# TheAustinator/keypoint-consensus-motion-correction

Hardware: AMD Instinct MI355X
Metric: aligned frames/sec (whole node) at 1080p; RANSAC hypotheses scored/sec/GPU (higher is better)
Workload: dtype u16 frames; u8 descriptors: i8 MFMA exact integer distances, f64 RANSAC, f32 warp weights

## Files before the change

keypoint-consensus-motion-correction_amd/csrc/ransac.hip:

```cpp
#include <cfloat>
#include <cmath>

#include "kcmc_internal.h"
#include "ransac_common.h"

namespace kcmc {
namespace {

using namespace ransac_common;

struct Model {
  double c, s, tx, ty;
  bool ok;
};

template <bool SCALE>
__device__ __forceinline__ Model fit2(double sx0, double sy0, double sx1, double sy1, double dx0, double dy0,
                                      double dx1, double dy1) {
  Model m;
  const double ms0 = (sx0 + sx1) / 2.0, ms1 = (sy0 + sy1) / 2.0;
  const double md0 = (dx0 + dx1) / 2.0, md1 = (dy0 + dy1) / 2.0;
  const double a0 = sx0 - ms0, a1 = sy0 - ms1, b0 = sx1 - ms0, b1 = sy1 - ms1;
  const double p0 = dx0 - md0, p1 = dy0 - md1, q0 = dx1 - md0, q1 = dy1 - md1;
  const double a00 = p0 * a0 + q0 * b0;
  const double a01 = p0 * a1 + q0 * b1;
  const double a10 = p1 * a0 + q1 * b0;
  const double a11 = p1 * a1 + q1 * b1;
  const double a = a00 + a11, b = a10 - a01;
  m.ok = !(a == 0.0 && b == 0.0);
  if (SCALE) {
    const double v = (a0 * a0 + b0 * b0) + (a1 * a1 + b1 * b1);
    m.c = a / v;
    m.s = b / v;
  } else {
    const double hn = sqrt(a * a + b * b);
    m.c = a / hn;
    m.s = b / hn;
  }
  m.tx = md0 - (m.c * ms0 - m.s * ms1);
  m.ty = md1 - (m.s * ms0 + m.c * ms1);
  return m;
}

struct Pts {
  const double* sx;
  const double* sy;
  const double* dx;
  const double* dy;
};

__device__ __forceinline__ double resid2(const Model& m, const Pts& P, int k, double thresh, int& cnt) {
  const double x = P.sx[k], y = P.sy[k];
  const double xp = fma(y, -m.s, x * m.c) + m.tx;
  const double yp = fma(y, m.c, x * m.s) + m.ty;
  const double ex = xp - P.dx[k], ey = yp - P.dy[k];
  const double r = sqrt_resid(ex * ex + ey * ey);
  cnt += (r < thresh) ? 1 : 0;
  return r * r;
}

__device__ __forceinline__ float score_fast(const Model& m, const Pts& P, int N, double tq, int& cnt) {
  float S = 0.f;
  for (int k = 0; k < N; ++k) {
    const double x = P.sx[k], y = P.sy[k];
    const double xp = fma(y, -m.s, x * m.c) + m.tx;
    const double yp = fma(y, m.c, x * m.s) + m.ty;
    const double ex = xp - P.dx[k], ey = yp - P.dy[k];
    const double q = ex * ex + ey * ey;
    cnt += (q < tq) ? 1 : 0;
    S += (float)q;
  }
  return S;
}

template <bool LARGE, bool SCALE>
__device__ __forceinline__ void ransac_rigid_frame(
    int f, const double* __restrict__ src, const double* __restrict__ dst, const int32_t* __restrict__ pt_idx,
    const int32_t* __restrict__ pt_off, int src_stride, const uint32_t* __restrict__ hyp,
    const int32_t* __restrict__ hyp_off, int hyp_off_len,
    int T, double thresh, double tq, double rate, int n_skip, double* __restrict__ out_params,
    uint8_t* __restrict__ out_inl, int32_t* __restrict__ out_nin, int32_t* __restrict__ out_best) {
  extern __shared__ __attribute__((aligned(16))) double smem[];
  __shared__ double red[kThreads / 64 * 8];
  __shared__ Scratch sc;
  __shared__ int s_any_zero;
  __shared__ Plan s_plan;

  const int tid = threadIdx.x;
  const int lane = tid & 63, wave = tid >> 6;
  int p0, N, hoff;
  if (!frame_begin<LARGE, 6>(f, pt_off, n_skip, 3, hyp_off, hyp_off_len, out_params, out_inl, out_nin, out_best, p0, N,
                             hoff))
    return;
  const uint32_t* H = hyp + hoff;

  double* sx = smem;
  double* sy = sx + N;
  double* dxs = sy + N;
  double* dys = dxs + N;
  float4* pk32 = reinterpret_cast<float4*>(dys + N);
  double* tS = reinterpret_cast<double*>(pk32 + N);
  double* tSh = tS + T;
  double* stk = tSh + T;
  double* wvals = stk + (LARGE ? kMaxStack * kThreads : 0);
  int* tC = reinterpret_cast<int*>(wvals + kThreads / 64 * 128);
  uint8_t* inl = reinterpret_cast<uint8_t*>(tC + T);
  if (LARGE && tid == 0) {
    s_plan.n = 0;
    plan_gen<kPwDepth>(s_plan, 0, N);
  }

  auto gather = [&](int k, double (&c)[4]) {
    gather_point(src, dst, pt_idx, src_stride, f, p0 + k, c[0], c[1], c[2], c[3]);
  };
  if (tid == 0) s_any_zero = 0;
  __shared__ Mag mg;
  if (!LARGE) {
    if (wave == 0) {
      double c[2][4], lo[4] = {INFINITY, INFINITY, INFINITY, INFINITY}, hi[4] = {-INFINITY, -INFINITY, -INFINITY, -INFINITY};
      bool bad = false;
#pragma unroll
      for (int h = 0; h < 2; ++h) {
        const int k = lane + 64 * h;
        if (k < N) {
          gather(k, c[h]);
          mag_add(c[h], lo, hi, bad);
        }
      }
      wave_bounds(lo, hi, bad);
      const Mag m = mag_of(lo, hi);
      if (lane == 0) mg = m;
#pragma unroll
      for (int h = 0; h < 2; ++h) {
        const int k = lane + 64 * h;
        if (k < N) {
          sx[k] = c[h][0];
          sy[k] = c[h][1];
          dxs[k] = c[h][2];
          dys[k] = c[h][3];
          pk32[k] = centred32(c[h][0], c[h][1], c[h][2], c[h][3], m);
        }
      }
    }
    __syncthreads();
  } else {
    for (int k = tid; k < N; k += kThreads) {
      double c[4];
      gather(k, c);
      sx[k] = c[0];
      sy[k] = c[1];
      dxs[k] = c[2];
      dys[k] = c[3];
    }
    __syncthreads();
    frame_mag(sx, sy, dxs, dys, N, red, mg);
    for (int k = tid; k < N; k += kThreads) pk32[k] = centred32(sx[k], sy[k], dxs[k], dys[k], mg);
    __syncthreads();
  }

  const Pts P{sx, sy, dxs, dys};
  auto fit_of = [&](int t) {
    const uint32_t pr = H[t];
    const int i = (int)(pr & 0xffffu), j = (int)(pr >> 16);
    return fit2<SCALE>(sx[i], sy[i], sx[j], sy[j], dxs[i], dys[i], dxs[j], dys[j]);
  };

  const bool fast = tq == tq;
  int mcount = -1, flag = fast ? 0 : 1;
  if (fast) {
    int mlo = -1;
    bool deferred = false;
    for (int t = tid; t < T; t += kThreads) {
      const Model m = fit_of(t);
      int v = -1;
      double slo = NAN, shi = NAN;
      Lin32 L;
      if (m.ok && lin32_make(m.c, -m.s, m.tx, m.s, m.c, m.ty, mg, tq, L)) {
        int clo = 0, chi = 0;
        const float S32 = score32(pk32, N, L, clo, chi);
        s32_bracket(S32, N, L.be, slo, shi);
        v = pack_cnt(clo, chi - clo);
        if (!(slo >= 1e-30 && shi <= 1e30)) flag = 1;
      } else if (m.ok) {
        v = INT_MIN;
        deferred = true;
      }
      tC[t] = v;
      tS[t] = slo;
      tSh[t] = shi;
      mlo = max(mlo, cnt_of(v));
    }
    if (deferred) {
      for (int t = tid; t < T; t += kThreads) {
        if (tC[t] != INT_MIN) continue;
        const Model m = fit_of(t);
        int cnt = 0;
        const float S32 = score_fast(m, P, N, tq, cnt);
        double slo, shi;
        s64_bracket(S32, N, slo, shi);
        if (!(slo >= 1e-30 && shi <= 1e30)) flag = 1;
        tC[t] = cnt;
        tS[t] = slo;
        tSh[t] = shi;
        mlo = max(mlo, cnt);
      }
    }
    block_max_flag(mlo, flag, sc.cnt);
    __syncthreads();
    for_each_wave_trial(
        T, [&](int t) { return !flag && und_of(tC[t]) > 0 && cnt_of(tC[t]) + und_of(tC[t]) >= mlo; },
        [&](int tc) {
          const Model m = fit_of(tc);
          int c = 0;
          double sq = 0.0;
          for (int k = lane; k < N; k += 64) {
            const double x = sx[k], y = sy[k];
            const double xp = fma(y, -m.s, x * m.c) + m.tx;
            const double yp = fma(y, m.c, x * m.s) + m.ty;
            const double ex = xp - dxs[k], ey = yp - dys[k];
            const double q = ex * ex + ey * ey;
            c += (q < tq) ? 1 : 0;
            sq += q;
          }
          c = wave_sum_i(c);
          double slo, shi;
          sd_bracket(wave_sum(sq), N, slo, shi);
          if (!(slo >= 1e-30 && shi <= 1e30)) flag = 1;
          if (lane == 0) {
            tC[tc] = c;
            tS[tc] = slo;
            tSh[tc] = shi;
          }
        });
    __syncthreads();
    for (int t = tid; t < T; t += kThreads) mcount = max(mcount, cnt_of(tC[t]));
  }
  block_max_flag(mcount, flag, sc.cnt);
  const bool exact = flag != 0 || mcount <= 0;

  Best best;
  bool any_zero = false;
  if (exact) {
    exact_trials(
        T,
        [&](int t, int& cnt) {
          const Model m = fit_of(t);
          if (!m.ok) return (double)NAN;
          return thread_pairwise<LARGE>([&](int k) { return resid2(m, P, k, thresh, cnt); }, N, s_plan, stk, tid);
        },
        tS, tC, best, any_zero);
  } else {
    double lm = INFINITY;
    for (int t = tid; t < T; t += kThreads)
      if (cnt_of(tC[t]) == mcount) lm = fmin(lm, tSh[t]);
    const double minhi = block_min(lm, sc.min);
    double* vals = wvals + wave * 128;
    double* wstk = stk + wave * kMaxStack;
    for_each_wave_trial(
        T, [&](int t) { return cnt_of(tC[t]) == mcount && tS[t] <= minhi; },
        [&](int tc) {
          const Model m = fit_of(tc);
          const double S = wave_pairwise<LARGE>(
              [&](int k) {
                int c = 0;
                return resid2(m, P, k, thresh, c);
              },
              N, s_plan, vals, wstk, lane);
          if (!isnan(S)) best.take(mcount, S, tc);
        });
  }
  int best_t, best_c;
  select_best(best, any_zero, T, tS, tC, sc, s_any_zero, best_t, best_c);

  Model bm{0, 0, 0, 0, false};
  if (best_t >= 0) bm = fit_of(best_t);
  for (int k = tid; k < N; k += kThreads) {
    int c = 0;
    if (bm.ok) resid2(bm, P, k, thresh, c);
    inl[k] = (uint8_t)c;
    out_inl[p0 + k] = (uint8_t)c;
  }
  __syncthreads();
  double n_in, ms0, ms1, md0, md1, a00 = 0, a01 = 0, a10 = 0, a11 = 0, vs = 0;
  if (!LARGE) {
    if (wave != 0) return;
    const int k1 = lane + 64;
    const bool i0 = lane < N && inl[lane], i1 = k1 < N && inl[k1];
    auto half_sums = [&](double lo, double hi) {
      for (int o = 32; o > 0; o >>= 1) {
        lo += __shfl_xor(lo, o);
        hi += __shfl_xor(hi, o);
      }
      return (((0.0 + lo) + hi) + 0.0) + 0.0;
    };
    n_in = half_sums(i0 ? 1.0 : 0.0, i1 ? 1.0 : 0.0);
    ms0 = half_sums(i0 ? 0.0 + sx[lane] : 0.0, i1 ? 0.0 + sx[k1] : 0.0) / n_in;
    ms1 = half_sums(i0 ? 0.0 + sy[lane] : 0.0, i1 ? 0.0 + sy[k1] : 0.0) / n_in;
    md0 = half_sums(i0 ? 0.0 + dxs[lane] : 0.0, i1 ? 0.0 + dxs[k1] : 0.0) / n_in;
    md1 = half_sums(i0 ? 0.0 + dys[lane] : 0.0, i1 ? 0.0 + dys[k1] : 0.0) / n_in;
    double b[2][4] = {{0, 0, 0, 0}, {0, 0, 0, 0}}, bv[2] = {0, 0};
#pragma unroll
    for (int h = 0; h < 2; ++h) {
      const int k = h ? k1 : lane;
      if (h ? i1 : i0) {
        const double u0 = sx[k] - ms0, u1 = sy[k] - ms1;
        const double v0 = dxs[k] - md0, v1 = dys[k] - md1;
        b[h][0] = 0.0 + v0 * u0;
        b[h][1] = 0.0 + v0 * u1;
        b[h][2] = 0.0 + v1 * u0;
        b[h][3] = 0.0 + v1 * u1;
        if (SCALE) bv[h] = 0.0 + (u0 * u0 + u1 * u1);
      }
    }
    a00 = half_sums(b[0][0], b[1][0]);
    a01 = half_sums(b[0][1], b[1][1]);
    a10 = half_sums(b[0][2], b[1][2]);
    a11 = half_sums(b[0][3], b[1][3]);
    if (SCALE) vs = half_sums(bv[0], bv[1]);
  } else {
    double s0 = 0, s1 = 0, s2 = 0, s3 = 0, cntd = 0;
    for (int k = tid; k < N; k += kThreads)
      if (inl[k]) {
        s0 += sx[k];
        s1 += sy[k];
        s2 += dxs[k];
        s3 += dys[k];
        cntd += 1.0;
      }
    n_in = block_sum(cntd, red);
    ms0 = block_sum(s0, red) / n_in;
    ms1 = block_sum(s1, red) / n_in;
    md0 = block_sum(s2, red) / n_in;
    md1 = block_sum(s3, red) / n_in;
    for (int k = tid; k < N; k += kThreads)
      if (inl[k]) {
        const double u0 = sx[k] - ms0, u1 = sy[k] - ms1;
        const double v0 = dxs[k] - md0, v1 = dys[k] - md1;
        a00 += v0 * u0;
        a01 += v0 * u1;
        a10 += v1 * u0;
        a11 += v1 * u1;
        if (SCALE) vs += u0 * u0 + u1 * u1;
      }
    a00 = block_sum(a00, red);
    a01 = block_sum(a01, red);
    a10 = block_sum(a10, red);
    a11 = block_sum(a11, red);
    if (SCALE) vs = block_sum(vs, red);
  }
  if (tid == 0) {
    double* o = out_params + 6 * (size_t)f;
    const double a = a00 + a11, b = a10 - a01;
    if (n_in > 0.0 && !(a == 0.0 && b == 0.0)) {
      const double hn = SCALE ? vs : sqrt(a * a + b * b);
      const double c = a / hn, s = b / hn;
      o[0] = c;
      o[1] = -s;
      o[2] = (md0 - (c * ms0 - s * ms1)) * rate;
      o[3] = s;
      o[4] = c;
      o[5] = (md1 - (s * ms0 + c * ms1)) * rate;
    } else {
      for (int k = 0; k < 6; ++k) o[k] = NAN;
    }
    out_nin[f] = (int32_t)n_in;
    out_best[f] = best_t;
  }
}

template <bool LARGE, bool SCALE>
__global__ __launch_bounds__(kThreads, 4) void ransac_rigid_kernel(
    const double* __restrict__ src, const double* __restrict__ dst, const int32_t* __restrict__ pt_idx,
    const int32_t* __restrict__ pt_off, int src_stride, const uint32_t* __restrict__ hyp,
    const int32_t* __restrict__ hyp_off, int hyp_off_len,
    int T, double thresh, double tq, double rate, int n_skip, double* __restrict__ out_params,
    uint8_t* __restrict__ out_inl, int32_t* __restrict__ out_nin, int32_t* __restrict__ out_best) {
  ransac_rigid_frame<LARGE, SCALE>(blockIdx.x, src, dst, pt_idx, pt_off, src_stride, hyp, hyp_off, hyp_off_len, T, thresh,
                                   tq, rate, n_skip, out_params, out_inl, out_nin, out_best);
}

}
}

using namespace kcmc;

template <bool SCALE>
static int ransac_rigid_impl(kcmc_ctx* ctx, const double* src, const double* dst, const int32_t* pt_idx,
                             const int32_t* pt_off, int src_frame_stride, int n_frames, int max_n, int trials,
                             double thresh, double rate, int n_skip, double* out_params, uint8_t* out_inliers,
                             int32_t* out_n_inliers, int32_t* out_best_trial, kcmc_stream_t stream) {
  const char* const who = SCALE ? "kcmc_ransac_similarity: " : "kcmc_ransac_rigid: ";
  const int rc = check_ransac_args(who, ctx, src, dst, pt_idx, pt_off, src_frame_stride, n_frames, max_n, trials,
                                   out_params, out_inliers, out_n_inliers, out_best_trial);
  if (rc != KCMC_OK || n_frames == 0) return rc;
  const int need = max_n < 3 ? 3 : max_n;
  if (!ctx->hyp || ctx->hyp_trials != trials)
    return fail(KCMC_EINVAL, std::string(who) + "hypothesis tables not prepared for trials=" +
                                 std::to_string(trials) + " (call kcmc_ransac_prepare)");
  const int n_small = need < 128 ? need : 128;
  const size_t wvals = (size_t)kThreads / 64 * 128 * sizeof(double);
  const size_t lds_small = (size_t)n_small * (4 * sizeof(double) + 16) + (size_t)trials * (2 * sizeof(double) + sizeof(int)) +
                           wvals + (size_t)n_small + 16;
  const size_t lds_large = (size_t)need * (4 * sizeof(double) + 16) + (size_t)trials * (2 * sizeof(double) + sizeof(int)) +
                           (size_t)kMaxStack * kThreads * sizeof(double) + wvals + (size_t)need + 16;
  return launch_small_large(who, ransac_rigid_kernel<false, SCALE>, ransac_rigid_kernel<true, SCALE>, n_frames, max_n,
                            lds_small, lds_large, (hipStream_t)stream, src, dst, pt_idx, pt_off, src_frame_stride,
                            ctx->hyp, ctx->hyp_off, ctx->hyp_off_len, trials, thresh, inlier_bound(thresh), rate, n_skip,
                            out_params, out_inliers, out_n_inliers, out_best_trial);
}

extern "C" int kcmc_ransac_rigid(kcmc_ctx* ctx, const double* src, const double* dst, const int32_t* pt_idx,
                                 const int32_t* pt_off, int src_frame_stride, int n_frames, int max_n, int trials,
                                 double thresh, double rate, int n_skip, double* out_params, uint8_t* out_inliers,
                                 int32_t* out_n_inliers, int32_t* out_best_trial, kcmc_stream_t stream) {
  return ransac_rigid_impl<false>(ctx, src, dst, pt_idx, pt_off, src_frame_stride, n_frames, max_n, trials, thresh, rate,
                                  n_skip, out_params, out_inliers, out_n_inliers, out_best_trial, stream);
}

extern "C" int kcmc_ransac_similarity(kcmc_ctx* ctx, const double* src, const double* dst, const int32_t* pt_idx,
                                      const int32_t* pt_off, int src_frame_stride, int n_frames, int max_n, int trials,
                                      double thresh, double rate, int n_skip, double* out_params, uint8_t* out_inliers,
                                      int32_t* out_n_inliers, int32_t* out_best_trial, kcmc_stream_t stream) {
  return ransac_rigid_impl<true>(ctx, src, dst, pt_idx, pt_off, src_frame_stride, n_frames, max_n, trials, thresh, rate,
                                 n_skip, out_params, out_inliers, out_n_inliers, out_best_trial, stream);
}
```

keypoint-consensus-motion-correction_amd/csrc/ransac_common.h:

```cpp
#pragma once

#include <climits>
#include <cmath>
#include <cstdint>

#include "kcmc_internal.h"

namespace kcmc {
namespace ransac_common {

constexpr int kThreads = 256;
constexpr int kMaxN = 4096;
constexpr int kPwDepth = 6;

constexpr int kMaxLeaves = 128;
constexpr int kMaxStack = kPwDepth + 2;

struct Plan {
  int16_t start[kMaxLeaves];
  int16_t len[kMaxLeaves];
  int8_t pops[kMaxLeaves];
  int n;
};

template <int DEPTH>
__device__ __forceinline__ void plan_gen(Plan& p, int s, int n) {
  if (DEPTH == 0 || n <= 128) {
    p.start[p.n] = (int16_t)s;
    p.len[p.n] = (int16_t)n;
    p.pops[p.n] = 0;
    ++p.n;
    return;
  }
  if constexpr (DEPTH > 0) {
    int n2 = n / 2;
    n2 -= n2 % 8;
    plan_gen<DEPTH - 1>(p, s, n2);
    plan_gen<DEPTH - 1>(p, s + n2, n - n2);
    ++p.pops[p.n - 1];
  }
}

__device__ __forceinline__ double sqrt_resid(double d) {
  const double y = __builtin_amdgcn_rsq(fmax(d, 0x1p-1000));
  double g = d * y;
  double h = y * 0.5;
  const double r = fma(-h, g, 0.5);
  g = fma(g, r, g);
  h = fma(h, r, h);
  double e = fma(-g, g, d);
  g = fma(e, h, g);
  e = fma(-g, g, d);
  return fma(e, h, g);
}

__device__ __forceinline__ bool better(int c, double S, int t, int bc, double bS, int bt) {
  if (c != bc) return c > bc;
  if (S != bS) return S < bS;
  return t < bt;
}

inline double inlier_bound(double thresh) {
  if (!(thresh > 0x1p-380 && thresh < 0x1p500)) return NAN;
  double q = thresh * thresh;
  while (std::sqrt(q) < thresh) q = std::nextafter(q, INFINITY);
  for (double p = std::nextafter(q, 0.0); std::sqrt(p) >= thresh; p = std::nextafter(q, 0.0)) q = p;
  return q;
}

template <class R2>
__device__ __forceinline__ double wave_leaf(R2 r2, int start, int n, double* vals, int lane) {
  for (int k = lane; k < n; k += 64) vals[k] = r2(start + k);
  __builtin_amdgcn_fence(__ATOMIC_RELEASE, "wavefront");
  __builtin_amdgcn_wave_barrier();
  __builtin_amdgcn_fence(__ATOMIC_ACQUIRE, "wavefront");
  double res = 0.0;
  if (n < 8) {
    for (int i = 0; i < n; ++i) res += vals[i];
  } else {
    const int j = lane & 7;
    const int nfull = n - (n % 8);
    double r = vals[j];
    for (int i = j + 8; i < nfull; i += 8) r += vals[i];
    double rj[8];
#pragma unroll
    for (int q = 0; q < 8; ++q) rj[q] = __shfl(r, q);
    res = ((rj[0] + rj[1]) + (rj[2] + rj[3])) + ((rj[4] + rj[5]) + (rj[6] + rj[7]));
    for (int i = nfull; i < n; ++i) res += vals[i];
  }
  __builtin_amdgcn_fence(__ATOMIC_RELEASE, "wavefront");
  __builtin_amdgcn_wave_barrier();
  __builtin_amdgcn_fence(__ATOMIC_ACQUIRE, "wavefront");
  return res;
}

template <bool LARGE, class R2>
__device__ __forceinline__ double wave_pairwise(R2 r2, int N, const Plan& plan, double* vals, double* wstk, int lane) {
  if (!LARGE) return wave_leaf(r2, 0, N, vals, lane);
  int sp = 0;
  for (int l = 0; l < plan.n; ++l) {
    wstk[sp++] = wave_leaf(r2, plan.start[l], plan.len[l], vals, lane);
    for (int c = plan.pops[l]; c > 0; --c) {
      const double b = wstk[--sp];
      const double a = wstk[sp - 1];
      wstk[sp - 1] = a + b;
    }
  }
  return wstk[0];
}

__device__ __forceinline__ double s32_eps(int N) { return (double)(N + 2) * 0x1p-22; }
__device__ __forceinline__ bool s32_certain(float S32) { return S32 >= 1e-30f && S32 <= 1e30f; }
__device__ __forceinline__ double sd_eps(int N) { return (double)(2 * N + 8) * 0x1p-52; }
__device__ __forceinline__ bool sd_certain(double Sd) { return Sd >= 1e-290 && Sd <= 1e290; }

typedef float f32x2 __attribute__((ext_vector_type(2)));

struct Mag {
  double cx, cy, cu, cv;
  double hx, hy, hu, hv;
  double X, Y, U, V;
};

struct Lin32 {
  f32x2 a, b, t;
  float lo, hi;
  double be;
};

__device__ __forceinline__ bool lin32_make(double ax, double bx, double tx, double ay, double by, double ty,
                                           const Mag& mg, double tq, Lin32& L) {
  const double tpx = ax * mg.cx + bx * mg.cy + tx - mg.cu;
  const double tpy = ay * mg.cx + by * mg.cy + ty - mg.cv;
  const double Mx = fabs(ax) * mg.hx + fabs(bx) * mg.hy + fabs(tpx) + mg.hu;
  const double My = fabs(ay) * mg.hx + fabs(by) * mg.hy + fabs(tpy) + mg.hv;
  const double Fx = fabs(ax) * mg.X + fabs(bx) * mg.Y + fabs(tx) + mg.U;
  const double Fy = fabs(ay) * mg.X + fabs(by) * mg.Y + fabs(ty) + mg.V;
  const double be = 7.01 * 0x1p-24 * fmax(Mx, My) + 0x1p-49 * fmax(Fx, Fy);
  const double B = 1.25 * (2.0 * be * sqrt(8.0 * tq) + 2.0 * be * be + 8.5 * 0x1p-24 * tq);
  if (!(B <= 0.25 * tq) || !(tq < 1e30)) return false;
  L.a = f32x2{(float)ax, (float)ay};
  L.b = f32x2{(float)bx, (float)by};
  L.t = f32x2{(float)tpx, (float)tpy};
  float lo = (float)(tq - B), hi = (float)(tq + B);
  if ((double)lo > tq - B) lo = __int_as_float(__float_as_int(lo) - 1);
  if ((double)hi < tq + B) hi = __int_as_float(__float_as_int(hi) + 1);
  L.lo = lo;
  L.hi = hi;
  L.be = be;
  return true;
}

__device__ __forceinline__ float4 centred32(double x, double y, double u, double v, const Mag& mg) {
  return make_float4((float)(x - mg.cx), (float)(y - mg.cy), (float)(u - mg.cu), (float)(v - mg.cv));
}

__device__ __forceinline__ float score32(const float4* __restrict__ pk, int N, const Lin32& L, int& clo, int& chi) {
  float S = 0.f;
  auto one = [&](const float4 p) {
    f32x2 e = L.t - f32x2{p.z, p.w};
    e = __builtin_elementwise_fma(L.b, f32x2{p.y, p.y}, e);
    e = __builtin_elementwise_fma(L.a, f32x2{p.x, p.x}, e);
    const float q = __builtin_fmaf(e.x, e.x, e.y * e.y);
    S += q;
    clo += q < L.lo ? 1 : 0;
    chi += q <= L.hi ? 1 : 0;
  };
  int k = 0;
  for (; k + 2 <= N; k += 2) {
    const float4 a = pk[k], b = pk[k + 1];
    one(a);
    one(b);
  }
  if (k < N) one(pk[k]);
  return S;
}

__device__ __forceinline__ void s32_bracket(float S32, int N, double be, double& lo, double& hi) {
  const double S = (double)S32;
  const double Sp = S * (1.0 + 1.01 * N * 0x1p-24);
  const double E = 2.0 * be * sqrt(2.02 * N * Sp) + 2.0 * N * be * be + ((N + 2.1) * 0x1p-24 + (N + 3) * 0x1p-53) * Sp;
  lo = (S - E) * (1.0 - 1e-9);
  hi = (S + E) * (1.0 + 1e-9);
}

__device__ __forceinline__ void s64_bracket(float S32, int N, double& lo, double& hi) {
  const double eps = s32_eps(N);
  lo = (double)S32 * (1.0 - eps);
  hi = (double)S32 * (1.0 + eps);
}

__device__ __forceinline__ void sd_bracket(double Sd, int N, double& lo, double& hi) {
  const double eps = (double)(2 * N + 8) * 0x1p-52;
  lo = Sd * (1.0 - eps);
  hi = Sd * (1.0 + eps);
}

__device__ __forceinline__ int pack_cnt(int cnt, int und) { return cnt | (und << 16); }
__device__ __forceinline__ int cnt_of(int v) { return v < 0 ? v : (v & 0xffff); }
__device__ __forceinline__ int und_of(int v) { return v < 0 ? 0 : (v >> 16); }

__device__ __forceinline__ int wave_sum_i(int v) {
  for (int o = 32; o > 0; o >>= 1) v += __shfl_xor(v, o);
  return v;
}

__device__ __forceinline__ Mag mag_of(const double (&L)[4], const double (&Hh)[4]) {
  double c[4], h[4], m[4];
#pragma unroll
  for (int i = 0; i < 4; ++i) {
    const bool fin = fabs(L[i]) < INFINITY && fabs(Hh[i]) < INFINITY;
    c[i] = fin ? 0.5 * L[i] + 0.5 * Hh[i] : 0.0;
    h[i] = fin ? fmax(Hh[i] - c[i], c[i] - L[i]) * (1.0 + 0x1p-50) : INFINITY;
    m[i] = fmax(fabs(L[i]), fabs(Hh[i]));
  }
  Mag out;
  out.cx = c[0]; out.cy = c[1]; out.cu = c[2]; out.cv = c[3];
  out.hx = h[0]; out.hy = h[1]; out.hu = h[2]; out.hv = h[3];
  out.X = m[0]; out.Y = m[1]; out.U = m[2]; out.V = m[3];
  return out;
}

__device__ __forceinline__ void mag_add(const double (&c)[4], double (&lo)[4], double (&hi)[4], bool& bad) {
#pragma unroll
  for (int i = 0; i < 4; ++i) {
    bad |= !(fabs(c[i]) < INFINITY);
    lo[i] = fmin(lo[i], c[i]);
    hi[i] = fmax(hi[i], c[i]);
  }
}

__device__ __forceinline__ void wave_bounds(double (&lo)[4], double (&hi)[4], bool bad) {
#pragma unroll
  for (int i = 0; i < 4; ++i) {
    if (bad) {
      lo[i] = -INFINITY;
      hi[i] = INFINITY;
    }
    for (int o = 32; o > 0; o >>= 1) {
      lo[i] = fmin(lo[i], __shfl_xor(lo[i], o));
      hi[i] = fmax(hi[i], __shfl_xor(hi[i], o));
    }
  }
}

__device__ inline void frame_mag(const double* sx, const double* sy, const double* dx, const double* dy, int N,
                                 double* red, Mag& out) {
  double lo[4] = {INFINITY, INFINITY, INFINITY, INFINITY}, hi[4] = {-INFINITY, -INFINITY, -INFINITY, -INFINITY};
  bool bad = false;
  for (int k = threadIdx.x; k < N; k += kThreads) {
    const double c[4] = {sx[k], sy[k], dx[k], dy[k]};
    mag_add(c, lo, hi, bad);
  }
  wave_bounds(lo, hi, bad);
  const int lane = threadIdx.x & 63, wave = threadIdx.x >> 6;
  __syncthreads();
  if (lane == 0)
#pragma unroll
    for (int i = 0; i < 4; ++i) {
      red[8 * wave + i] = lo[i];
      red[8 * wave + 4 + i] = hi[i];
    }
  __syncthreads();
  double L[4], Hh[4];
#pragma unroll
  for (int i = 0; i < 4; ++i) {
    L[i] = red[i];
    Hh[i] = red[4 + i];
    for (int w = 1; w < kThreads / 64; ++w) {
      L[i] = fmin(L[i], red[8 * w + i]);
      Hh[i] = fmax(Hh[i], red[8 * w + 4 + i]);
    }
  }
  if (threadIdx.x == 0) out = mag_of(L, Hh);
  __syncthreads();
}

__device__ inline double block_sum(double v, double* red) {
  for (int o = 32; o > 0; o >>= 1) v += __shfl_xor(v, o);
  const int lane = threadIdx.x & 63, wave = threadIdx.x >> 6;
  __syncthreads();
  if (lane == 0) red[wave] = v;
  __syncthreads();
  double s = 0.0;
  for (int w = 0; w < kThreads / 64; ++w) s += red[w];
  return s;
}

__device__ __forceinline__ double wave_sum(double v) {
  for (int o = 32; o > 0; o >>= 1) v += __shfl_xor(v, o);
  return v;
}


struct Scratch {
  double min[kThreads / 64];
  double bestS[kThreads / 64];
  int cnt[kThreads / 64];
  int best[kThreads / 64 * 2];
};

template <bool LARGE, int NPARAM>
__device__ __forceinline__ bool frame_begin(int f, const int32_t* __restrict__ pt_off, int n_skip, int min_n,
                                            const int32_t* __restrict__ hyp_off, int hyp_off_len,
                                            double* __restrict__ out_params, uint8_t* __restrict__ out_inl,
                                            int32_t* __restrict__ out_nin, int32_t* __restrict__ out_best, int& p0,
                                            int& N, int& hoff) {
  const int tid = threadIdx.x;
  p0 = pt_off[f];
  N = pt_off[f + 1] - p0;
  const bool skip_frame = N < n_skip || N < min_n || N > kMaxN;
  hoff = (!skip_frame && N < hyp_off_len) ? hyp_off[N] : -1;
  const bool nan_frame = skip_frame || hoff < 0;
  if (LARGE != (!nan_frame && N > 128)) return false;
  if (nan_frame) {
    if (tid < NPARAM) out_params[NPARAM * (size_t)f + tid] = NAN;
    for (int k = tid; k < N; k += kThreads) out_inl[p0 + k] = 0;
    if (tid == 0) {
      out_nin[f] = skip_frame ? 0 : -1;
      out_best[f] = -1;
    }
    return false;
  }
  return true;
}

__device__ __forceinline__ void gather_point(const double* __restrict__ src, const double* __restrict__ dst,
                                             const int32_t* __restrict__ pt_idx, int src_stride, int f, int p,
                                             double& x, double& y, double& u, double& v) {
  size_t si, di;
  if (pt_idx) {
    const int q = pt_idx[p];
    si = (size_t)f * src_stride + q;
    di = (size_t)q;
  } else {
    si = di = (size_t)p;
  }
  x = src[2 * si];
  y = src[2 * si + 1];
  u = dst[2 * di];
  v = dst[2 * di + 1];
}

__device__ __forceinline__ void block_max_flag(int& m, int& flag, int* s_cnt) {
  for (int o = 32; o > 0; o >>= 1) {
    m = max(m, __shfl_xor(m, o));
    flag |= __shfl_xor(flag, o);
  }
  if ((threadIdx.x & 63) == 0) s_cnt[threadIdx.x >> 6] = (m + 1) | (flag << 30);
  __syncthreads();
#pragma unroll
  for (int w = 0; w < kThreads / 64; ++w) {
    const int v = s_cnt[w];
    flag |= v >> 30;
    m = max(m, (v & 0x3fffffff) - 1);
  }
}

__device__ __forceinline__ double block_min(double v, double* s_min) {
  for (int o = 32; o > 0; o >>= 1) v = fmin(v, __shfl_xor(v, o));
  if ((threadIdx.x & 63) == 0) s_min[threadIdx.x >> 6] = v;
  __syncthreads();
  return fmin(fmin(s_min[0], s_min[1]), fmin(s_min[2], s_min[3]));
}

template <class R2>
__device__ __forceinline__ double pw_leaf(R2 r2, int start, int n) {
  if (n < 8) {
    double res = 0.0;
    for (int i = 0; i < n; ++i) res += r2(start + i);
    return res;
  }
  double r[8];
#pragma unroll
  for (int j = 0; j < 8; ++j) r[j] = r2(start + j);
  int i = 8;
  const int nfull = n - (n % 8);
  for (; i < nfull; i += 8) {
#pragma unroll
    for (int j = 0; j < 8; ++j) r[j] += r2(start + i + j);
  }
  double res = ((r[0] + r[1]) + (r[2] + r[3])) + ((r[4] + r[5]) + (r[6] + r[7]));
  for (; i < n; ++i) res += r2(start + i);
  return res;
}

template <bool LARGE, class R2>
__device__ __forceinline__ double thread_pairwise(R2 r2, int N, const Plan& plan, double* stk, int tid) {
  if (!LARGE) return pw_leaf(r2, 0, N);
  int sp = 0;
  for (int l = 0; l < plan.n; ++l) {
    stk[sp++ * kThreads + tid] = pw_leaf(r2, plan.start[l], plan.len[l]);
    for (int c = plan.pops[l]; c > 0; --c) {
      const double b = stk[--sp * kThreads + tid];
      const double a = stk[(sp - 1) * kThreads + tid];
      stk[(sp - 1) * kThreads + tid] = a + b;
    }
  }
  return stk[tid];
}

struct Best {
  int c = -1;
  double S = INFINITY;
  int t = INT_MAX;
  __device__ __forceinline__ void take(int oc, double oS, int ot) {
    if (better(oc, oS, ot, c, S, t)) {
      c = oc;
      S = oS;
      t = ot;
    }
  }
};

template <class Score>
__device__ __forceinline__ void exact_trials(int T, Score score, double* tS, int* tC, Best& best, bool& any_zero) {
  for (int t = threadIdx.x; t < T; t += kThreads) {
    int cnt = 0;
    const double S = score(t, cnt);
    tS[t] = S;
    tC[t] = cnt;
    if (!isnan(S) && (cnt > 0 || S < INFINITY)) {
      if (S <= 0.0) any_zero = true;
      best.take(cnt, S, t);
    }
  }
}

template <class Pred, class Body>
__device__ __forceinline__ void for_each_wave_trial(int T, Pred pred, Body body) {
  const int lane = threadIdx.x & 63, wave = threadIdx.x >> 6;
  for (int t0 = wave * 64; t0 < T; t0 += kThreads) {
    const int t = t0 + lane;
    uint64_t todo = __ballot(t < T && pred(t));
    while (todo) {
      const int tc = t0 + __builtin_ctzll(todo);
      todo &= todo - 1;
      body(tc);
    }
  }
}

__device__ __forceinline__ void select_best(Best b, bool any_zero, int T, const double* tS, const int* tC, Scratch& sc,
                                            int& s_any_zero, int& best_t, int& best_c) {
  const int tid = threadIdx.x;
  const int lane = tid & 63, wave = tid >> 6;
  for (int o = 32; o > 0; o >>= 1) b.take(__shfl_xor(b.c, o), __shfl_xor(b.S, o), __shfl_xor(b.t, o));
  if (lane == 0) {
    sc.best[2 * wave] = b.c;
    sc.best[2 * wave + 1] = b.t;
    sc.bestS[wave] = b.S;
  }
  if (any_zero) atomicOr(&s_any_zero, 1);
  __syncthreads();
  if (tid == 0) {
    Best fin;
    for (int w = 0; w < kThreads / 64; ++w) fin.take(sc.best[2 * w], sc.bestS[w], sc.best[2 * w + 1]);
    if (s_any_zero) {
      int c0 = 0, t0 = -1;
      double S0 = INFINITY;
      for (int t = 0; t < T; ++t) {
        const double S = tS[t];
        const int c = tC[t];
        if (isnan(S)) continue;
        if (c > c0 || (c == c0 && S < S0)) {
          c0 = c;
          S0 = S;
          t0 = t;
          if (S0 <= 0.0) break;
        }
      }
      fin.t = t0 < 0 ? INT_MAX : t0;
      fin.c = c0;
    }
    sc.best[0] = (fin.t == INT_MAX) ? -1 : fin.t;
    sc.best[1] = (fin.t == INT_MAX) ? 0 : fin.c;
  }
  __syncthreads();
  best_t = sc.best[0];
  best_c = sc.best[1];
}

inline int check_ransac_args(const char* who, const kcmc_ctx* ctx, const double* src, const double* dst,
                             const int32_t* pt_idx, const int32_t* pt_off, int src_frame_stride, int n_frames,
                             int max_n, int trials, const double* out_params, const uint8_t* out_inliers,
                             const int32_t* out_n_inliers, const int32_t* out_best_trial) {
  if (!ctx) return fail(KCMC_EINVAL, std::string(who) + "ctx is NULL");
  if (n_frames < 0 || max_n < 0 || trials < 1) return fail(KCMC_EINVAL, std::string(who) + "bad sizes");
  if (n_frames == 0) return KCMC_OK;
  if (!pt_off || !out_params || !out_n_inliers || !out_best_trial || (max_n > 0 && (!src || !dst || !out_inliers)))
    return fail(KCMC_EINVAL, std::string(who) + "NULL pointer");
  if (max_n > kMaxN) return fail(KCMC_EUNSUPPORTED, std::string(who) + "max_n > 4096 points per frame");
  if (pt_idx && src_frame_stride <= 0) return fail(KCMC_EINVAL, std::string(who) + "src_frame_stride must be > 0");
  return KCMC_OK;
}

template <class... P, class... A>
inline int launch_small_large(const char* who, void (*small)(P...), void (*large)(P...), int n_frames, int max_n,
                              size_t lds_small, size_t lds_large, hipStream_t s, A... args) {
  if ((max_n > 128 ? lds_large : lds_small) > 150 * 1024)
    return fail(KCMC_EUNSUPPORTED, std::string(who) + "max_n/trials exceed the LDS budget");
  hipLaunchKernelGGL(small, dim3((unsigned)n_frames), dim3(kThreads), lds_small, s, args...);
  KCMC_TRY(launch_check((std::string(who) + "small scoring kernel").c_str()));
  if (max_n > 128) {
    hipLaunchKernelGGL(large, dim3((unsigned)n_frames), dim3(kThreads), lds_large, s, args...);
    KCMC_TRY(launch_check((std::string(who) + "large scoring kernel").c_str()));
  }
  return KCMC_OK;
}

}
}
```

Before: 624,000.

## Compress small-N rigid RANSAC trial records to cut LDS and raise occupancy

For the N<=128 rigid RANSAC kernel, per-trial records go from a packed int count plus two double score brackets to u8 count and undecided fields plus float brackets rounded outward. The small-path LDS regions are overlaid with a union-like layout, so the exact-path tS/tC and the wave scratch reuse the fast-path space and the pk32 buffer. Together with launch bounds raised from 4 to 5 blocks per SIMD, this aims to fit more workgroups per CU. The costs are more complex layout aliasing and float-rounded brackets that loosen pruning slightly. The any_zero/NaN handling in exact_trials and select_best also changes.

```diff
diff --git a/keypoint-consensus-motion-correction_amd/csrc/ransac.hip b/keypoint-consensus-motion-correction_amd/csrc/ransac.hip
--- a/keypoint-consensus-motion-correction_amd/csrc/ransac.hip
+++ b/keypoint-consensus-motion-correction_amd/csrc/ransac.hip
@@ -99,12 +99,55 @@
   double* dxs = sy + N;
   double* dys = dxs + N;
   float4* pk32 = reinterpret_cast<float4*>(dys + N);
-  double* tS = reinterpret_cast<double*>(pk32 + N);
+  double* tS = reinterpret_cast<double*>(pk32 + (LARGE ? N : 0));
   double* tSh = tS + T;
   double* stk = tSh + T;
-  double* wvals = stk + (LARGE ? kMaxStack * kThreads : 0);
-  int* tC = reinterpret_cast<int*>(wvals + kThreads / 64 * 128);
-  uint8_t* inl = reinterpret_cast<uint8_t*>(tC + T);
+  double* wvals = LARGE ? stk + kMaxStack * kThreads : tS;
+  int* tC = reinterpret_cast<int*>(LARGE ? wvals + kThreads / 64 * 128 : tS + T);
+  float* fLo = reinterpret_cast<float*>(tS + 4 * N);
+  float* fHi = fLo + T;
+  uint8_t* bC = reinterpret_cast<uint8_t*>(fHi + T);
+  uint8_t* bU = bC + T;
+  uint8_t* inl = LARGE ? reinterpret_cast<uint8_t*>(tC + T)
+                       : reinterpret_cast<uint8_t*>(tS) + max(32 * N + 10 * T, 12 * T);
+  auto rec_put = [&](int t, int v, double slo, double shi) {
+    if constexpr (LARGE) {
+      tC[t] = v;
+      tS[t] = slo;
+      tSh[t] = shi;
+    } else {
+      bC[t] = v == INT_MIN ? kDeferred : v < 0 ? kNoModel : (uint8_t)(v & 0xffff);
+      bU[t] = (uint8_t)und_of(v);
+      fLo[t] = (float)slo;
+      fHi[t] = (float)shi;
+    }
+  };
+  auto outward = [&](double& slo, double& shi) {
+    if constexpr (!LARGE) {
+      slo = (double)f32_below(slo);
+      shi = (double)f32_above(shi);
+    }
+  };
+  auto rec_cnt = [&](int t) {
+    if constexpr (LARGE) return cnt_of(tC[t]);
+    else return cnt_of8(bC[t]);
+  };
+  auto rec_und = [&](int t) {
+    if constexpr (LARGE) return und_of(tC[t]);
+    else return bC[t] >= kDeferred ? 0 : (int)bU[t];
+  };
+  auto rec_deferred = [&](int t) {
+    if constexpr (LARGE) return tC[t] == INT_MIN;
+    else return bC[t] == kDeferred;
+  };
+  auto rec_lo = [&](int t) {
+    if constexpr (LARGE) return tS[t];
+    else return (double)fLo[t];
+  };
+  auto rec_hi = [&](int t) {
+    if constexpr (LARGE) return tSh[t];
+    else return (double)fHi[t];
+  };
   if (LARGE && tid == 0) {
     s_plan.n = 0;
     plan_gen<kPwDepth>(s_plan, 0, N);
@@ -179,36 +222,34 @@
         int clo = 0, chi = 0;
         const float S32 = score32(pk32, N, L, clo, chi);
         s32_bracket(S32, N, L.be, slo, shi);
+        outward(slo, shi);
         v = pack_cnt(clo, chi - clo);
         if (!(slo >= 1e-30 && shi <= 1e30)) flag = 1;
       } else if (m.ok) {
         v = INT_MIN;
         deferred = true;
       }
-      tC[t] = v;
-      tS[t] = slo;
-      tSh[t] = shi;
+      rec_put(t, v, slo, shi);
       mlo = max(mlo, cnt_of(v));
     }
     if (deferred) {
       for (int t = tid; t < T; t += kThreads) {
-        if (tC[t] != INT_MIN) continue;
+        if (!rec_deferred(t)) continue;
         const Model m = fit_of(t);
         int cnt = 0;
         const float S32 = score_fast(m, P, N, tq, cnt);
         double slo, shi;
         s64_bracket(S32, N, slo, shi);
+        outward(slo, shi);
         if (!(slo >= 1e-30 && shi <= 1e30)) flag = 1;
-        tC[t] = cnt;
-        tS[t] = slo;
-        tSh[t] = shi;
+        rec_put(t, cnt, slo, shi);
         mlo = max(mlo, cnt);
       }
     }
     block_max_flag(mlo, flag, sc.cnt);
     __syncthreads();
     for_each_wave_trial(
-        T, [&](int t) { return !flag && und_of(tC[t]) > 0 && cnt_of(tC[t]) + und_of(tC[t]) >= mlo; },
+        T, [&](int t) { return !flag && rec_und(t) > 0 && rec_cnt(t) + rec_und(t) >= mlo; },
         [&](int tc) {
           const Model m = fit_of(tc);
           int c = 0;
@@ -225,15 +266,12 @@
           c = wave_sum_i(c);
           double slo, shi;
           sd_bracket(wave_sum(sq), N, slo, shi);
+          outward(slo, shi);
           if (!(slo >= 1e-30 && shi <= 1e30)) flag = 1;
-          if (lane == 0) {
-            tC[tc] = c;
-            tS[tc] = slo;
-            tSh[tc] = shi;
-          }
+          if (lane == 0) rec_put(tc, c, slo, shi);
         });
     __syncthreads();
-    for (int t = tid; t < T; t += kThreads) mcount = max(mcount, cnt_of(tC[t]));
+    for (int t = tid; t < T; t += kThreads) mcount = max(mcount, rec_cnt(t));
   }
   block_max_flag(mcount, flag, sc.cnt);
   const bool exact = flag != 0 || mcount <= 0;
@@ -252,12 +290,12 @@
   } else {
     double lm = INFINITY;
     for (int t = tid; t < T; t += kThreads)
-      if (cnt_of(tC[t]) == mcount) lm = fmin(lm, tSh[t]);
+      if (rec_cnt(t) == mcount) lm = fmin(lm, rec_hi(t));
     const double minhi = block_min(lm, sc.min);
-    double* vals = wvals + wave * 128;
+    double* vals = wvals + wave * (LARGE ? 128 : N);
     double* wstk = stk + wave * kMaxStack;
     for_each_wave_trial(
-        T, [&](int t) { return cnt_of(tC[t]) == mcount && tS[t] <= minhi; },
+        T, [&](int t) { return rec_cnt(t) == mcount && rec_lo(t) <= minhi; },
         [&](int tc) {
           const Model m = fit_of(tc);
           const double S = wave_pairwise<LARGE>(
@@ -369,7 +407,7 @@
 }
 
 template <bool LARGE, bool SCALE>
-__global__ __launch_bounds__(kThreads, 4) void ransac_rigid_kernel(
+__global__ __launch_bounds__(kThreads, LARGE ? 4 : 5) void ransac_rigid_kernel(
     const double* __restrict__ src, const double* __restrict__ dst, const int32_t* __restrict__ pt_idx,
     const int32_t* __restrict__ pt_off, int src_stride, const uint32_t* __restrict__ hyp,
     const int32_t* __restrict__ hyp_off, int hyp_off_len,
@@ -378,6 +416,9 @@
   ransac_rigid_frame<LARGE, SCALE>(blockIdx.x, src, dst, pt_idx, pt_off, src_stride, hyp, hyp_off, hyp_off_len, T, thresh,
                                    tq, rate, n_skip, out_params, out_inl, out_nin, out_best);
 }
+
+static_assert(rigid_small_lds(128, 1000) + sizeof(Scratch) + sizeof(Mag) + 16 <= 20480,
+              "the N <= 128 rigid RANSAC workgroup must fit one warp tile's LDS");
 
 }
 }
@@ -399,8 +440,7 @@
                                  std::to_string(trials) + " (call kcmc_ransac_prepare)");
   const int n_small = need < 128 ? need : 128;
   const size_t wvals = (size_t)kThreads / 64 * 128 * sizeof(double);
-  const size_t lds_small = (size_t)n_small * (4 * sizeof(double) + 16) + (size_t)trials * (2 * sizeof(double) + sizeof(int)) +
-                           wvals + (size_t)n_small + 16;
+  const size_t lds_small = rigid_small_lds((size_t)n_small, (size_t)trials);
   const size_t lds_large = (size_t)need * (4 * sizeof(double) + 16) + (size_t)trials * (2 * sizeof(double) + sizeof(int)) +
                            (size_t)kMaxStack * kThreads * sizeof(double) + wvals + (size_t)need + 16;
   return launch_small_large(who, ransac_rigid_kernel<false, SCALE>, ransac_rigid_kernel<true, SCALE>, n_frames, max_n,
diff --git a/keypoint-consensus-motion-correction_amd/csrc/ransac_common.h b/keypoint-consensus-motion-correction_amd/csrc/ransac_common.h
--- a/keypoint-consensus-motion-correction_amd/csrc/ransac_common.h
+++ b/keypoint-consensus-motion-correction_amd/csrc/ransac_common.h
@@ -196,6 +196,28 @@
   hi = Sd * (1.0 + eps);
 }
 
+__host__ __device__ inline float f32_step(float f, bool up) {
+  int32_t i = __builtin_bit_cast(int32_t, f);
+  if (f == 0.f) return __builtin_bit_cast(float, up ? 0x00000001 : (int32_t)0x80000001);
+  i += ((f > 0.f) == up) ? 1 : -1;
+  return __builtin_bit_cast(float, i);
+}
+__host__ __device__ inline float f32_below(double d) {
+  const float f = (float)d;
+  return (double)f > d ? f32_step(f, false) : f;
+}
+__host__ __device__ inline float f32_above(double d) {
+  const float f = (float)d;
+  return (double)f < d ? f32_step(f, true) : f;
+}
+
+constexpr uint8_t kNoModel = 255, kDeferred = 254;
+__host__ __device__ inline int cnt_of8(uint8_t c) { return c >= kDeferred ? -1 : (int)c; }
+constexpr size_t rigid_small_lds(size_t n, size_t T) {
+  const size_t fast = 32 * n + 10 * T, exact = 12 * T;
+  return 32 * n + (fast > exact ? fast : exact) + n + 16;
+}
+
 __device__ __forceinline__ int pack_cnt(int cnt, int und) { return cnt | (und << 16); }
 __device__ __forceinline__ int cnt_of(int v) { return v < 0 ? v : (v & 0xffff); }
 __device__ __forceinline__ int und_of(int v) { return v < 0 ? 0 : (v >> 16); }
@@ -423,6 +445,8 @@
     if (!isnan(S) && (cnt > 0 || S < INFINITY)) {
       if (S <= 0.0) any_zero = true;
       best.take(cnt, S, t);
+    } else if (cnt > 0) {
+      any_zero = true;
     }
   }
 }
@@ -462,7 +486,6 @@
       for (int t = 0; t < T; ++t) {
         const double S = tS[t];
         const int c = tC[t];
-        if (isnan(S)) continue;
         if (c > c0 || (c == c0 && S < S0)) {
           c0 = c;
           S0 = S;
```

After: 633,000 (median of 6 runs). 1.4% higher.
